# nanoporetech/taiyaki

Measured on AMD Instinct MI355X. Metric: signal-chunks/sec (T=4000) flip-flop train step, higher is better.
Workload: dtype f32; 1 GPU; configs[1]: mLstm_flipflop r9.4.1 DNA, chunk_len=4000 (T=800 blocks), 128 chunks/GPU, size 256, HIP flip-flop CRF loss + logZ, gradient maxima/clipping, AdamW; config_id=2, model=mLstm_flipflop, global_batch=128, chunk_len=4000, launch=hipGraph replay of forward+loss and of AdamW, eager backward, hw_queues=4, conv=gemm, lstm=miopen, batches=pre-assembled, cycled from HBM, parallelism=dp1 (reads sharded; one flat RCCL gradient all-reduce after backward)

## Files before the change

taiyaki_amd/csrc/lstm_fwd_layout.h:

```cpp
#pragma once

namespace tk {

constexpr bool lstm_fwd_lanes(int H, int U, int C) { return H == 256 && U == 64 && C == 2; }

struct LstmFwdLanes {
    int NT, H, U, C;
    int KP, KS, PR, CK;

    constexpr LstmFwdLanes(int nt, int h, int u, int c)
        : NT(nt), H(h), U(u), C(c), KP(nt / u), KS(h * u / nt), PR(c < 4 ? 4 / c : 1), CK(4 * c * u / nt) {}

    constexpr bool ok() const {
        return KP * U == NT && KS * KP == H && KP >= 4 && KP <= 64 && (KP & (KP - 1)) == 0 && PR >= 1 &&
               (PR * C) % 4 == 0 && KS % PR == 0 && CK >= 1 && CK * KP == 4 * C && C % CK == 0;
    }
    constexpr int k(int kp, int i) const { return i * KP + kp; }
    constexpr int hs_index(int k_, int c) const {
        return ((k_ / KP / PR) * KP + k_ % KP) * PR * C + (k_ / KP % PR) * C + c;
    }
    constexpr int chunk(int kp, int j) const { return (j * KP + kp) * PR * C; }
    constexpr int flat(int gate, int c) const { return (c / CK) * 4 * CK + gate * CK + c % CK; }
    constexpr int kept_first(int kp) const {
        int a = 0, n = 4 * C;
        for (int m = 1; m < KP; m <<= 1) {
            n /= 2;
            if (kp & m) a += n;
        }
        return a;
    }
    constexpr int gate(int kp) const { return kept_first(kp) % (4 * CK) / CK; }
    constexpr int col(int kp, int v) const { return kept_first(kp) / (4 * CK) * CK + v; }
    constexpr bool cell_lane(int kp) const { return gate(kp) == 0; }
    constexpr int gate_lane_xor(int g) const {
        for (int x = 0; x < KP; ++x)
            if (gate(x) == g && col(x, 0) == 0) return x;
        return -1;
    }
};

}
```

taiyaki_amd/csrc/lstm_kernels.hip:

```cpp
#include "dispatch.h"
#include "ff_common.h"
#include "lstm_bwd_layout.h"
#include "lstm_fwd_layout.h"
#include "rnn_common.h"

namespace tk {
namespace {

template <int U>
constexpr int threads_for() { return U == 48 ? 384 : U <= 32 ? 256 : 512; }
template <int H, int U>
constexpr int bwd_threads_for() { return U == 48 ? 2 * H : threads_for<U>(); }

template <int M>
__device__ __forceinline__ float xor_lane(float v) {
    static_assert(M == 1 || M == 2 || M == 4, "a partner inside the lane's group of 8");
    const int x = __float_as_int(v);
    if constexpr (M == 1) {
        return __int_as_float(__builtin_amdgcn_update_dpp(0, x, 0xB1, 0xF, 0xF, true));
    } else if constexpr (M == 2) {
        return __int_as_float(__builtin_amdgcn_update_dpp(0, x, 0x4E, 0xF, 0xF, true));
    } else {
        const int y = __builtin_amdgcn_update_dpp(0, x, 0x141, 0xF, 0xF, true);
        return __int_as_float(__builtin_amdgcn_update_dpp(0, y, 0x1B, 0xF, 0xF, true));
    }
}

template <int M, int RQ, int NA>
__device__ __forceinline__ void halve_rounds(float (&acc)[NA], int rq) {
    if constexpr (M < RQ) {
        constexpr int n = NA / (2 * M);
        const bool up = (rq & M) != 0;
#pragma unroll
        for (int a = 0; a < n; ++a) {
            const float send = up ? acc[a] : acc[a + n];
            const float keep = up ? acc[a + n] : acc[a];
            acc[a] = keep + xor_lane<M>(send);
        }
        halve_rounds<2 * M, RQ>(acc, rq);
    }
}

template <int H, int C, int U, bool VL, bool SAVE>
__device__ __forceinline__ void lstm_fwd_lanes_body(const float *__restrict__ gx, const float *__restrict__ whh, int T,
                                                    Cols cols, int reverse, int ngroups, float *__restrict__ y,
                                                    float *__restrict__ gates, float *__restrict__ cell, u64 *hbuf,
                                                    uint32_t *status, const int32_t *__restrict__ lengths) {
    constexpr int NT = threads_for<U>();
    const int N = cols.n, LD = cols.ld();
    constexpr int G = H / U;
    constexpr LstmFwdLanes FL(NT, H, U, C);
    constexpr int KP = FL.KP, KS = FL.KS, PR = FL.PR, CK = FL.CK;
    constexpr int NG = H * C / NT;
    static_assert(FL.ok() && KP == 8 && NG * NT == H * C && FL.gate_lane_xor(1) == 4 && FL.gate_lane_xor(2) == 2 &&
                      FL.gate_lane_xor(3) == 6,
                  "whole rows in 16-byte reads; the partial sums and the four gates of a column inside 8 lanes of a wave");
    constexpr int U4 = U / 4;
    constexpr int NQ = SAVE ? (6 * C * U4 + NT - 1) / NT : 1;
    static_assert(U % 4 == 0, "a row of the staging block is whole 16-byte chunks");
    __shared__ __attribute__((aligned(16))) float hs[2][H * C];
    __shared__ __attribute__((aligned(16))) float stg[SAVE ? 2 : 1][SAVE ? 6 * C * U : 4];
    __shared__ int give_up;

    int group, member;
    place(G, group, member);
    const int tid = threadIdx.x;
    const int j0 = member * U, n0 = group * C;
    const int u = tid / KP, kp = tid % KP;

    float w[4][KS];
#pragma unroll
    for (int g = 0; g < 4; ++g)
#pragma unroll
        for (int i = 0; i < KS; ++i) w[g][i] = whh[((size_t)g * H + j0 + u) * H + FL.k(kp, i)];
    settle(w);

    const int gate = FL.gate(kp), col = FL.col(kp, 0);
    const bool cell_lane = gate == 0;
    const int n = n0 + col;
    bool fetch[CK], valid[CK];
    float cst[CK], held[CK];
    int len[CK];
#pragma unroll
    for (int v = 0; v < CK; ++v) {
        fetch[v] = n + v < N;
        valid[v] = cell_lane && fetch[v];
        cst[v] = held[v] = 0.f;
        len[v] = 0;
        if constexpr (VL) len[v] = !valid[v] ? 0 : lengths ? lengths[n + v] : T;
    }

    for (int i = tid; i < H * C; i += NT) hs[0][i] = 0.f;
    if (tid == 0) give_up = 0;

    const size_t H4 = 4 * (size_t)H;
    float *rp[NQ];
    size_t rpitch[NQ];
    if constexpr (SAVE) {
#pragma unroll
        for (int i = 0; i < NQ; ++i) {
            const int q = tid + i * NT, row = q / U4, v = row / C, nn = n0 + row % C;
            const size_t w = v < 2 ? (size_t)H : H4;
            float *base = v == 0 ? y : v == 1 ? cell : gates + (size_t)(v - 2) * H;
            rpitch[i] = (size_t)LD * w;
            rp[i] = q < 6 * C * U4 && nn < N ? base + (size_t)nn * w + j0 + 4 * (q % U4) : nullptr;
        }
    }
    const float *gx0 = gx + (size_t)n * H4 + (size_t)gate * H + j0 + u;
    float gq[CK];
#pragma unroll
    for (int v = 0; v < CK; ++v) gq[v] = fetch[v] ? gx0[(size_t)(reverse ? T - 1 : 0) * LD * H4 + v * H4] : 0.f;
    __syncthreads();

    for (int s = 0; s < T; ++s) {
        const int t = reverse ? T - 1 - s : s;
        float *hb = hs[s & 1];
        settle(gq);
        if (s > 0) {
            const u64 *src = hbuf + ((size_t)((s - 1) & 1) * ngroups + group) * (H * C);
            float v[NG];
            if (!sweep<NG>(src, tid, NT, H * C, (unsigned)s, v, status)) give_up = 1;
#pragma unroll
            for (int q = 0; q < NG; ++q) {
                const int e = tid + q * NT;
                hb[FL.hs_index(e % H, e / H)] = v[q];
            }
            __syncthreads();
            if (give_up) return;
            const int tl = reverse ? t + 1 : t - 1;
            if constexpr (!SAVE) {
#pragma unroll
                for (int v = 0; v < CK; ++v)
                    if (valid[v]) y[((size_t)tl * LD + n + v) * H + j0 + u] = held[v];
            } else {
                rows_to_global<NQ>(stg[(s - 1) & 1], tid, NT, rp, rpitch, (size_t)tl);
            }
        }
        float gn[CK];
#pragma unroll
        for (int v = 0; v < CK; ++v)
            gn[v] = fetch[v] && s + 1 < T ? gx0[(size_t)(reverse ? t - 1 : t + 1) * LD * H4 + v * H4] : 0.f;
        asm volatile("" ::: "memory");

        float acc[4 * C];
#pragma unroll
        for (int a = 0; a < 4 * C; ++a) acc[a] = 0.f;
        constexpr int NR = KS / PR, AHEAD = 4;
        float hv[NR][PR * C];
#pragma unroll
        for (int j = 0; j < AHEAD; ++j) lds_row<PR * C>(hb + FL.chunk(kp, j), hv[j]);
#pragma unroll
        for (int j = 0; j < NR; ++j) {
            if (j + AHEAD < NR) lds_row<PR * C>(hb + FL.chunk(kp, j + AHEAD), hv[j + AHEAD]);
            __builtin_amdgcn_sched_barrier(0);
#pragma unroll
            for (int e = 0; e < PR; ++e)
#pragma unroll
                for (int g = 0; g < 4; ++g)
#pragma unroll
                    for (int c = 0; c < C; ++c)
                        acc[FL.flat(g, c)] = fmaf(w[g][PR * j + e], hv[j][e * C + c], acc[FL.flat(g, c)]);
        }
        halve_rounds<1, KP>(acc, kp);

        float ig[CK], fg[CK], gg[CK], og[CK];
#pragma unroll
        for (int v = 0; v < CK; ++v) {
            const float x = acc[v] + gq[v];
            float a;
            if (gate == 2)
                a = tanhf(x);
            else
                a = sigmoidf(x);
            ig[v] = a;
            gg[v] = xor_lane<2>(a);
            fg[v] = xor_lane<4>(a);
            og[v] = xor_lane<2>(fg[v]);
        }

        if (cell_lane) {
            float h[CK];
#pragma unroll
            for (int v = 0; v < CK; ++v) {
                cst[v] = fmaf(ig[v], gg[v], fg[v] * cst[v]);
                h[v] = og[v] * tanhf(cst[v]);
                if constexpr (VL) {
                    if (t >= len[v]) {
                        cst[v] = h[v] = 0.f;
                        if constexpr (SAVE) ig[v] = fg[v] = gg[v] = og[v] = 0.f;
                    }
                }
            }
            if (s + 1 < T) {
#pragma unroll
                for (int v = 0; v < CK; ++v)
                    store_granule(hbuf + ((size_t)(s & 1) * ngroups + group) * (H * C) + (col + v) * H + j0 + u,
                                  (unsigned)(s + 1), h[v]);
            }
#pragma unroll
            for (int v = 0; v < CK; ++v) {
                if constexpr (!SAVE) {
                    held[v] = h[v];
                } else {
                    float *sp = stg[s & 1] + (col + v) * U + u;
                    sp[0 * C * U] = h[v];
                    sp[1 * C * U] = cst[v];
                    sp[2 * C * U] = ig[v];
                    sp[3 * C * U] = fg[v];
                    sp[4 * C * U] = gg[v];
                    sp[5 * C * U] = og[v];
                }
            }
        }
#pragma unroll
        for (int v = 0; v < CK; ++v) gq[v] = gn[v];
    }
    if (T > 0) {
        const int tl = reverse ? 0 : T - 1;
        if constexpr (!SAVE) {
#pragma unroll
            for (int v = 0; v < CK; ++v)
                if (valid[v]) y[((size_t)tl * LD + n + v) * H + j0 + u] = held[v];
        } else {
            __syncthreads();
            rows_to_global<NQ>(stg[(T - 1) & 1], tid, NT, rp, rpitch, (size_t)tl);
        }
    }
}

template <int H, int C, int U, bool VL = false, bool SAVE = !VL>
__global__ __launch_bounds__(threads_for<U>(), 1) void lstm_fwd_kernel(const float *__restrict__ gx,
                                                                       const float *__restrict__ whh, int T, Cols cols,
                                                                       int reverse, int ngroups,
                                                                       float *__restrict__ y,
                                                                       float *__restrict__ gates,
                                                                       float *__restrict__ cell, u64 *hbuf,
                                                                       uint32_t *status,
                                                                       const int32_t *__restrict__ lengths) {
    if constexpr (lstm_fwd_lanes(H, U, C)) {
        lstm_fwd_lanes_body<H, C, U, VL, SAVE>(gx, whh, T, cols, reverse, ngroups, y, gates, cell, hbuf, status, lengths);
        return;
    }
    constexpr int NT = threads_for<U>();
    const int N = cols.n, LD = cols.ld();
    constexpr int G = H / U;
    constexpr int KP = NT / U;
    constexpr int KS = H / KP;
    constexpr int NG = (H * C + NT - 1) / NT;
    static_assert(KS >= 1 && KP <= 64 && C <= KP, "lane (u, kp) inside one wave; one cell lane per (u, column)");
    constexpr int U4 = U / 4;
    constexpr int NQ = SAVE ? (6 * C * U4 + NT - 1) / NT : 1;
    static_assert(U % 4 == 0, "a row of the staging block is whole 16-byte chunks");
    __shared__ __attribute__((aligned(16))) float hs[2][H * C];
    __shared__ __attribute__((aligned(16))) float stg[SAVE ? 2 : 1][SAVE ? 6 * C * U : 4];
    __shared__ int give_up;

    int group, member;
    place(G, group, member);
    const int tid = threadIdx.x;
    const int j0 = member * U, n0 = group * C;
    const int u = tid / KP, kp = tid % KP;

    float w[4][KS];
#pragma unroll
    for (int g = 0; g < 4; ++g)
#pragma unroll
        for (int i = 0; i < KS; ++i) w[g][i] = whh[((size_t)g * H + j0 + u) * H + i * KP + kp];
    settle(w);

    int col = 0;
#pragma unroll
    for (int m = 1, width = C; width > 1; m <<= 1, width >>= 1)
        if (kp & m) col += width / 2;
    const bool cell_lane = kp < C;
    const int n = n0 + col;
    const bool valid = cell_lane && n < N;
    float cst = 0.f;
    int len = 0;
    if constexpr (VL) len = !valid ? 0 : lengths ? lengths[n] : T;

    for (int i = tid; i < H * C; i += NT) hs[0][i] = 0.f;
    if (tid == 0) give_up = 0;

    const size_t H4 = 4 * (size_t)H;
    float *rp[NQ];
    size_t rpitch[NQ];
    if constexpr (SAVE) {
#pragma unroll
        for (int i = 0; i < NQ; ++i) {
            const int q = tid + i * NT, row = q / U4, v = row / C, nn = n0 + row % C;
            const size_t w = v < 2 ? (size_t)H : H4;
            float *base = v == 0 ? y : v == 1 ? cell : gates + (size_t)(v - 2) * H;
            rpitch[i] = (size_t)LD * w;
            rp[i] = q < 6 * C * U4 && nn < N ? base + (size_t)nn * w + j0 + 4 * (q % U4) : nullptr;
        }
    }
    float gq[4] = {0.f, 0.f, 0.f, 0.f};
    if (valid) {
        const float *p = gx + ((size_t)(reverse ? T - 1 : 0) * LD + n) * H4 + j0 + u;
#pragma unroll
        for (int g = 0; g < 4; ++g) gq[g] = p[(size_t)g * H];
    }
    float held = 0.f;
    __syncthreads();

    for (int s = 0; s < T; ++s) {
        const int t = reverse ? T - 1 - s : s;
        float *hb = hs[s & 1];
        settle(gq);
        if (s > 0) {
            const u64 *src = hbuf + ((size_t)((s - 1) & 1) * ngroups + group) * (H * C);
            float v[NG];
            if (!sweep<NG>(src, tid, NT, H * C, (unsigned)s, v, status)) give_up = 1;
#pragma unroll
            for (int q = 0; q < NG; ++q) {
                const int e = tid + q * NT;
                if (e < H * C) hb[(e % H) * C + e / H] = v[q];
            }
            __syncthreads();
            if (give_up) return;
            const int tl = reverse ? t + 1 : t - 1;
            if constexpr (!SAVE) {
                if (valid) y[((size_t)tl * LD + n) * H + j0 + u] = held;
            } else {
                rows_to_global<NQ>(stg[(s - 1) & 1], tid, NT, rp, rpitch, (size_t)tl);
            }
        }
        float gn[4] = {0.f, 0.f, 0.f, 0.f};
        if (valid && s + 1 < T) {
            const float *p = gx + ((size_t)(reverse ? t - 1 : t + 1) * LD + n) * H4 + j0 + u;
#pragma unroll
            for (int g = 0; g < 4; ++g) gn[g] = p[(size_t)g * H];
        }
        asm volatile("" ::: "memory");

        float acc[4][C];
#pragma unroll
        for (int g = 0; g < 4; ++g)
#pragma unroll
            for (int c = 0; c < C; ++c) acc[g][c] = 0.f;
#pragma unroll
        for (int i = 0; i < KS; ++i) {
            float hv[C];
            lds_row<C>(hb + (i * KP + kp) * C, hv);
#pragma unroll
            for (int g = 0; g < 4; ++g)
#pragma unroll
                for (int c = 0; c < C; ++c) acc[g][c] = fmaf(w[g][i], hv[c], acc[g][c]);
        }
#pragma unroll
        for (int m = 1; m < KP; m <<= 1) {
            const int half = C / (2 * m);
            const bool up = (kp & m) != 0;
#pragma unroll
            for (int g = 0; g < 4; ++g) {
                if (half == 0) acc[g][0] += __shfl_xor(acc[g][0], m);
#pragma unroll
                for (int c = 0; c < C / 2; ++c) {
                    if (c < half) {
                        const float send = up ? acc[g][c] : acc[g][c + half];
                        const float keep = up ? acc[g][c + half] : acc[g][c];
                        acc[g][c] = keep + __shfl_xor(send, m);
                    }
                }
            }
        }

        if (cell_lane) {
            float ig = sigmoidf(acc[0][0] + gq[0]), fg = sigmoidf(acc[1][0] + gq[1]);
            float gg = tanhf(acc[2][0] + gq[2]), og = sigmoidf(acc[3][0] + gq[3]);
            cst = fmaf(ig, gg, fg * cst);
            float h = og * tanhf(cst);
            if constexpr (VL) {
                if (t >= len) {
                    cst = h = 0.f;
                    if constexpr (SAVE) ig = fg = gg = og = 0.f;
                }
            }
            if (s + 1 < T)
                store_granule(hbuf + ((size_t)(s & 1) * ngroups + group) * (H * C) + col * H + j0 + u,
                              (unsigned)(s + 1), h);
            if constexpr (!SAVE) {
                held = h;
            } else {
                float *sp = stg[s & 1] + col * U + u;
                sp[0 * C * U] = h;
                sp[1 * C * U] = cst;
                sp[2 * C * U] = ig;
                sp[3 * C * U] = fg;
                sp[4 * C * U] = gg;
                sp[5 * C * U] = og;
            }
        }
#pragma unroll
        for (int g = 0; g < 4; ++g) gq[g] = gn[g];
    }
    if (T > 0) {
        const int tl = reverse ? 0 : T - 1;
        if constexpr (!SAVE) {
            if (valid) y[((size_t)tl * LD + n) * H + j0 + u] = held;
        } else {
            __syncthreads();
            rows_to_global<NQ>(stg[(T - 1) & 1], tid, NT, rp, rpitch, (size_t)tl);
        }
    }
}

#ifndef TK_RNN_VARLEN
template <int H, int C, int U, bool VL = false>
__global__ __launch_bounds__((bwd_threads_for<H, U>()), 1) void lstm_bwd_kernel(const float *__restrict__ whh,
                                                                       const float *__restrict__ gates,
                                                                       const float *__restrict__ cell,
                                                                       const float *__restrict__ dy, int T, Cols cols,
                                                                       int reverse, int ngroups,
                                                                       float *__restrict__ dgates, u64 *pbuf,
                                                                       uint32_t *status,
                                                                       const int32_t *__restrict__ lengths) {
    constexpr int NT = bwd_threads_for<H, U>();
    const int N = cols.n, LD = cols.ld();
    constexpr int G = H / U;
    constexpr bool STRIDED = U == 48;
    constexpr int RP = NT / H;
    constexpr int R = 4 * U / RP;
    constexpr LstmBwdBlock LB(NT, H, U, C);
    constexpr bool BLOCK = LB.KQ > 0;
    constexpr int KQ = BLOCK ? LB.KQ : 1, RQ = BLOCK ? LB.RQ : 1, RR = BLOCK ? LB.RR : 1, KEEP = BLOCK ? LB.KEEP : 1;
    constexpr int PAIRS = U * C;
    constexpr int PL = NT / PAIRS;
    constexpr int NP = (G + PL - 1) / PL;
    constexpr bool APART = BLOCK && NP > 1;
    static_assert(!APART || NP * PL == G, "every plane polls NP producers");
    static_assert(RP >= 1 && R >= 1 && PL >= 1 && PL * PAIRS == NT, "every lane polls; one cell lane per pair");
    static_assert(!STRIDED || (RP * H == NT && R * RP == 4 * U && U % RP == 0),
                  "a lane's rows keep their gate index at compile time");
    static_assert(!BLOCK || (LB.ok() && KQ * RR * NT == 4 * U * H && RQ <= 64 && (RQ & (RQ - 1)) == 0 &&
                             KEEP * NT == C * H && KQ * RR == R),
                  "every owned weight in one lane; the RQ partial sums inside one wave; one granule per held sum");
    __shared__ __attribute__((aligned(16))) float dgs[4 * U * C];
    __shared__ float gath[(APART ? G : PL) * PAIRS];
    __shared__ __attribute__((aligned(16))) float red[RP > 1 && !BLOCK ? RP * C * H : 1];
    __shared__ int give_up;

    int group, member;
    place(G, group, member);
    const int tid = threadIdx.x;
    const int j0 = member * U, n0 = group * C;

    const int k = tid % H, rp = tid / H;
    const int kb = tid / RQ, rq = tid % RQ;
    float w[R];
    if constexpr (BLOCK) {
#pragma unroll
        for (int j = 0; j < RR; ++j) {
            const int r = LB.row(rq, j);
#pragma unroll
            for (int q = 0; q < KQ; ++q) w[q * RR + j] = whh[((size_t)(r / U) * H + j0 + (r % U)) * H + KQ * kb + q];
        }
    } else if constexpr (STRIDED) {
        const float *wbase = whh + (size_t)(j0 + rp) * H + k;
#pragma unroll
        for (int i = 0; i < R; ++i) w[i] = wbase[(unsigned)((((i * RP) / U) * H + (i * RP) % U) * H)];
    } else {
#pragma unroll
        for (int i = 0; i < R; ++i) {
            const int r = rp * R + i;
            w[i] = whh[((size_t)(r / U) * H + j0 + (r % U)) * H + k];
        }
    }
    settle(w);

    const bool cell_lane = tid < PAIRS;
    const int pair = tid % PAIRS, plane = tid / PAIRS;
    const int cc = pair / U, u = pair % U;
    const int n = n0 + cc;
    const bool valid = cell_lane && n < N;
    float dc_next = 0.f, f_next = 0.f;
    int len = 0;
    if constexpr (VL) len = !valid ? 0 : lengths ? lengths[n] : T;
    if (tid == 0) give_up = 0;

    const size_t H4 = 4 * (size_t)H;
    float in[7] = {0.f, 0.f, 0.f, 0.f, 0.f, 0.f, 0.f};
    if (valid) {
        const int t = reverse ? 0 : T - 1;
        const size_t o = ((size_t)t * LD + n) * H + j0 + u;
        in[0] = dy[o];
        in[1] = cell[o];
        if (T > 1) in[2] = cell[((size_t)(reverse ? t + 1 : t - 1) * LD + n) * H + j0 + u];
        const float *gp = gates + ((size_t)t * LD + n) * H4 + j0 + u;
#pragma unroll
        for (int g = 0; g < 4; ++g) in[3 + g] = gp[(size_t)g * H];
    }
    float held[4] = {0.f, 0.f, 0.f, 0.f};
    __syncthreads();

    const u64 *mine = pbuf + (size_t)group * G * C * H + cc * H + j0 + u;
    const int a0 = LB.kept_first(rq), pub = (a0 % C) * H + KQ * kb + a0 / C;
    for (int s = 0; s < T; ++s) {
        const int tt = T - 1 - s;
        const int t = reverse ? T - 1 - tt : tt;
        const int tp = reverse ? t + 1 : t - 1;
        settle(in);
        float dhr = 0.f;
        if (s > 0) {
            float v[NP];
            const int nvalid = plane < G ? (G - plane + PL - 1) / PL : 0;
            const u64 *src = mine + (size_t)((s - 1) & 1) * ngroups * G * C * H;
            if (!sweep<NP>(src, plane * C * H, PL * C * H, G * C * H, (unsigned)s, v, status)) give_up = 1;
            if constexpr (APART) {
#pragma unroll
                for (int q = 0; q < NP; ++q) gath[(plane + q * PL) * PAIRS + pair] = v[q];
            } else {
                float sum = 0.f;
#pragma unroll
                for (int q = 0; q < NP; ++q)
                    if (q < nvalid) sum += v[q];
                gath[plane * PAIRS + pair] = sum;
            }
            __syncthreads();
            if (give_up) return;
            if (cell_lane) {
#pragma unroll
                for (int p = 0; p < (APART ? G : PL); ++p) dhr += gath[p * PAIRS + pair];
            }
            if (valid) {
                const int tl = reverse ? t - 1 : t + 1;
                float *dp = dgates + ((size_t)tl * LD + n) * H4 + j0 + u;
#pragma unroll
                for (int g = 0; g < 4; ++g) dp[(size_t)g * H] = held[g];
            }
        }
        float nx[7] = {0.f, 0.f, 0.f, 0.f, 0.f, 0.f, 0.f};
        if (valid && tt > 0) {
            const size_t o = ((size_t)tp * LD + n) * H + j0 + u;
            nx[0] = dy[o];
            nx[1] = in[2];
            if (tt > 1) nx[2] = cell[((size_t)(reverse ? tp + 1 : tp - 1) * LD + n) * H + j0 + u];
            const float *gp = gates + ((size_t)tp * LD + n) * H4 + j0 + u;
#pragma unroll
            for (int g = 0; g < 4; ++g) nx[3 + g] = gp[(size_t)g * H];
        }
        asm volatile("" ::: "memory");

        if (cell_lane) {
            const float ct = in[1];
            float cp = in[2];
            if constexpr (VL) {
                if (tp >= len) cp = 0.f;
            }
            const float ig = in[3], gg = in[5], og = in[6];
            float fg = in[4];
            const float dh = in[0] + dhr;
            const float tc = tanhf(ct);
            float dc = dh * og * (1.f - tc * tc) + dc_next * f_next;
            float di = dc * gg * ig * (1.f - ig);
            float df = dc * cp * fg * (1.f - fg);
            float dg = dc * ig * (1.f - gg * gg);
            float dout = dh * tc * og * (1.f - og);
            if constexpr (VL) {
                if (t >= len) dc = fg = di = df = dg = dout = 0.f;
            }
            dc_next = dc;
            f_next = fg;
            held[0] = di;
            held[1] = df;
            held[2] = dg;
            held[3] = dout;
            dgs[(0 * U + u) * C + cc] = valid ? di : 0.f;
            dgs[(1 * U + u) * C + cc] = valid ? df : 0.f;
            dgs[(2 * U + u) * C + cc] = valid ? dg : 0.f;
            dgs[(3 * U + u) * C + cc] = valid ? dout : 0.f;
        }
#pragma unroll
        for (int q = 0; q < 7; ++q) in[q] = nx[q];
        __syncthreads();
        if (s + 1 == T) break;

        if constexpr (BLOCK) {
            u64 *dst = pbuf + (((size_t)(s & 1) * ngroups + group) * G + member) * C * H;
            float acc[KQ * C];
#pragma unroll
            for (int a = 0; a < KQ * C; ++a) acc[a] = 0.f;
#pragma unroll
            for (int i = 0; i < RR / 2; ++i) {
                float d[2 * C];
                lds_row<2 * C>(dgs + (rq + RQ * i) * 2 * C, d);
#pragma unroll
                for (int e = 0; e < 2; ++e)
#pragma unroll
                    for (int q = 0; q < KQ; ++q)
#pragma unroll
                        for (int c = 0; c < C; ++c)
                            acc[q * C + c] = fmaf(w[q * RR + 2 * i + e], d[e * C + c], acc[q * C + c]);
            }
            halve_rounds<1, RQ>(acc, rq);
#pragma unroll
            for (int v = 0; v < KEEP; ++v) store_granule(dst + pub + v * H, (unsigned)(s + 1), acc[v]);
            continue;
        }
        float acc[C];
#pragma unroll
        for (int c = 0; c < C; ++c) acc[c] = 0.f;
#pragma unroll
        for (int i = 0; i < R; ++i) {
            float d[C];
            lds_row<C>(dgs + (STRIDED ? i * RP + rp : rp * R + i) * C, d);
#pragma unroll
            for (int c = 0; c < C; ++c) acc[c] = fmaf(w[i], d[c], acc[c]);
        }
        u64 *dst = pbuf + (((size_t)(s & 1) * ngroups + group) * G + member) * C * H;
        if constexpr (RP == 1) {
#pragma unroll
            for (int c = 0; c < C; ++c) store_granule(dst + c * H + k, (unsigned)(s + 1), acc[c]);
        } else {
#pragma unroll
            for (int c = 0; c < C; ++c) red[(rp * C + c) * H + k] = acc[c];
            __syncthreads();
            for (int e = tid; e < C * H; e += NT) {
                float v = 0.f;
#pragma unroll
                for (int q = 0; q < RP; ++q) v += red[q * C * H + e];
                store_granule(dst + e, (unsigned)(s + 1), v);
            }
        }
    }
    if (valid && T > 0) {
        const int tl = reverse ? T - 1 : 0;
        float *dp = dgates + ((size_t)tl * LD + n) * H4 + j0 + u;
#pragma unroll
        for (int g = 0; g < 4; ++g) dp[(size_t)g * H] = held[g];
    }
}

#endif

int g_lab_cols = 0;
int g_lab_units = 0;

int units48(size_t H) { return H == 192 || H == 384 ? 48 : 0; }

bool lstm_geometry(size_t N, size_t H, int cu_count, int *C_out, int *groups_out) {
    const int U48 = units48(H);
    if (!(U48 || H == 16 || H == 32 || H == 64 || H == 128 || H == 256) || N == 0 || cu_count <= 0) return false;
    const size_t G = H / (U48 ? U48 : 16);
    const int first = U48 ? 4 : 8, last = H == 384 ? 4 : 2 * first;
    for (int C = first; C <= last; C *= 2) {
        if (g_lab_cols != 0 && C != g_lab_cols) continue;
        const size_t groups = (N + C - 1) / C;
        if (groups * G <= (size_t)cu_count) {
            *C_out = C;
            *groups_out = (int)groups;
            return true;
        }
    }
    return false;
}

size_t ws_bytes(size_t H, int C, int groups, int U, bool backward) {
    return 2 * (size_t)groups * (backward ? H / U : 1) * C * H * sizeof(u64);
}

struct Plan {
    int U, C, groups;
    unsigned grid;
};

bool lstm_plan(size_t N, size_t H, int cu_count, Plan *p) {
    int C16 = 0, groups16 = 0;
    if (!lstm_geometry(N, H, cu_count, &C16, &groups16)) return false;
    if (const int U48 = units48(H)) {
        *p = Plan{U48, C16, groups16, (unsigned)(groups16 * (H / U48))};
        return true;
    }
    int U = g_lab_units != 0 ? g_lab_units : 64;
    if ((size_t)U > H) U = (int)H;
    if (U != 16 && U != 32 && U != 64) return false;
    p->U = U;
    p->C = C16 * 16 / U;
    p->groups = (int)((N + p->C - 1) / p->C);
    p->grid = (unsigned)(p->groups * (H / U));
    return true;
}

#define TK_LSTM_SWITCH(LAUNCH)                                                                                    \
    switch ((int)H * 100000 + p.U * 1000 + p.C) {                                                                 \
        LAUNCH(16, 16, 8) LAUNCH(16, 16, 16) LAUNCH(32, 16, 8) LAUNCH(32, 16, 16) LAUNCH(64, 16, 8)                \
        LAUNCH(64, 16, 16) LAUNCH(128, 16, 8) LAUNCH(128, 16, 16) LAUNCH(256, 16, 8) LAUNCH(256, 16, 16)          \
        LAUNCH(32, 32, 4) LAUNCH(32, 32, 8) LAUNCH(64, 32, 4) LAUNCH(64, 32, 8) LAUNCH(128, 32, 4)                 \
        LAUNCH(128, 32, 8) LAUNCH(256, 32, 4) LAUNCH(256, 32, 8)                                                  \
        LAUNCH(64, 64, 2) LAUNCH(64, 64, 4) LAUNCH(128, 64, 2) LAUNCH(128, 64, 4) LAUNCH(256, 64, 2)               \
        LAUNCH(256, 64, 4) LAUNCH(192, 48, 4) LAUNCH(192, 48, 8) LAUNCH(384, 48, 4)                               \
        default: return TK_ERR_UNSUPPORTED;                                                                       \
    }

template <bool VL, bool SAVE>
int launch_fwd(const Plan &p, size_t H, hipStream_t st, const float *gx, const float *whh, int T, Cols cols,
               int rev, float *y, float *gates, float *cell, u64 *ws, uint32_t *status, const int32_t *lengths) {
#define TK_LSTM_FWD(HH, UU, CC)                                                                                  \
    case HH * 100000 + UU * 1000 + CC:                                                                           \
        hipLaunchKernelGGL((lstm_fwd_kernel<HH, CC, UU, VL, SAVE>), dim3(p.grid), dim3(threads_for<UU>()), 0, st, gx,  \
                           whh, T, cols, rev, p.groups, y, gates, cell, ws, status, lengths);                    \
        break;
    TK_LSTM_SWITCH(TK_LSTM_FWD)
#undef TK_LSTM_FWD
    return hipGetLastError() == hipSuccess ? TK_OK : TK_ERR_LAUNCH;
}

#ifndef TK_RNN_VARLEN
template <bool VL>
int launch_bwd(const Plan &p, size_t H, hipStream_t st, const float *whh, const float *gates, const float *cell,
               const float *dy, int T, Cols cols, int rev, float *dg, u64 *ws, uint32_t *status,
               const int32_t *lengths) {
#define TK_LSTM_BWD(HH, UU, CC)                                                                                   \
    case HH * 100000 + UU * 1000 + CC:                                                                            \
        hipLaunchKernelGGL((lstm_bwd_kernel<HH, CC, UU, VL>), dim3(p.grid), dim3(bwd_threads_for<HH, UU>()), 0,   \
                           st, whh, gates, cell, dy, T, cols, rev, p.groups, dg, ws, status, lengths);            \
        break;
    TK_LSTM_SWITCH(TK_LSTM_BWD)
#undef TK_LSTM_BWD
    return hipGetLastError() == hipSuccess ? TK_OK : TK_ERR_LAUNCH;
}
#endif
#undef TK_LSTM_SWITCH

size_t lstm_slab(size_t N, size_t H, int cu_count) {
    int C = 0, groups = 0;
    const size_t S = widest_admitted([&](size_t n) { return lstm_geometry(n, H, cu_count, &C, &groups); });
    return N == 0 ? 0 : N < S ? N : S;
}

template <class Launch>
int checked(bool pointers_ok, size_t T, size_t N, size_t H, int cu_count, void *ws, size_t wsb, uint32_t *status,
            hipStream_t stream, bool backward, Launch launch) {
    if (!pointers_ok || !ws || !status || !aligned16(ws) || T > (size_t)INT32_MAX || N > (size_t)INT32_MAX)
        return TK_ERR_BAD_ARG;
#ifdef TK_RNN_WIDE
    const size_t S = lstm_slab(N, H, cu_count);
#else
    const size_t S = N;
#endif
    if (S == 0) return TK_ERR_UNSUPPORTED;
    for (size_t first = 0; first < N; first += S) {
        const size_t n = N - first < S ? N - first : S;
        Plan p;
        if (!lstm_plan(n, H, cu_count, &p)) return TK_ERR_UNSUPPORTED;
        const size_t need = ws_bytes(H, p.C, p.groups, p.U, backward);
        if (wsb < need) return TK_ERR_WORKSPACE;
        if (T == 0) continue;
        int rc = zero_ws(ws, need, stream);
        if (rc != TK_OK) return rc;
        rc = launch(p, first, make_cols(n, N));
        if (rc != TK_OK) return rc;
    }
    return TK_OK;
}

size_t train_workspace_bytes(size_t N, size_t H, int cu_count) {
    int C = 0, groups = 0;
    if (!lstm_geometry(N, H, cu_count, &C, &groups)) return 0;
    const int U48 = units48(H);
    return ws_bytes(H, C, groups, U48 ? U48 : 16, true);
}

template <bool VL, bool SAVE>
int forward(const float *gx, const float *whh, const int32_t *lengths, size_t T, size_t N, size_t H, int reverse,
            int cu_count, float *y, float *gates, float *cell, void *ws, size_t wsb, uint32_t *status,
            hipStream_t stream) {
    auto launch = [&](const Plan &p, size_t first, Cols cols) {
        return launch_fwd<VL, SAVE>(p, H, stream, at_column(gx, first, 4 * H), whh, (int)T, cols, reverse,
                                    at_column(y, first, H), at_column(gates, first, 4 * H), at_column(cell, first, H),
                                    static_cast<u64 *>(ws), status, at_column(lengths, first, 1));
    };
    return checked(gx && whh && y && (!SAVE || (gates && cell)), T, N, H, cu_count, ws, wsb, status, stream, false,
                   launch);
}

#ifndef TK_RNN_VARLEN
template <bool VL>
int backward(const float *whh, const float *gates, const float *cell, const float *dy, const int32_t *lengths,
             size_t T, size_t N, size_t H, int reverse, int cu_count, float *dgates, void *ws, size_t wsb,
             uint32_t *status, hipStream_t stream) {
    auto launch = [&](const Plan &p, size_t first, Cols cols) {
        return launch_bwd<VL>(p, H, stream, whh, at_column(gates, first, 4 * H), at_column(cell, first, H),
                              at_column(dy, first, H), (int)T, cols, reverse, at_column(dgates, first, 4 * H),
                              static_cast<u64 *>(ws), status, at_column(lengths, first, 1));
    };
    return checked(whh && gates && cell && dy && dgates, T, N, H, cu_count, ws, wsb, status, stream, true, launch);
}
#endif

}

#ifdef TK_RNN_VARLEN
size_t lstm_varlen_workspace_bytes(size_t N, size_t H, int cu_count) {
    Plan p;
    if (!lstm_plan(N, H, cu_count, &p)) return 0;
    return ws_bytes(H, p.C, p.groups, p.U, false);
}

int lstm_forward_varlen_dispatch(const float *gx, const float *whh, const int32_t *lengths, size_t T, size_t N,
                                 size_t H, int reverse, int cu_count, float *y, void *ws, size_t wsb,
                                 uint32_t *status, hipStream_t stream) {
    return forward<true, false>(gx, whh, lengths, T, N, H, reverse, cu_count, y, nullptr, nullptr, ws, wsb, status,
                                stream);
}
#elif defined(TK_RNN_VARLEN_TRAIN)
size_t lstm_varlen_train_workspace_bytes(size_t N, size_t H, int cu_count) {
    return train_workspace_bytes(N, H, cu_count);
}

int lstm_forward_varlen_save_dispatch(const float *gx, const float *whh, const int32_t *lengths, size_t T, size_t N,
                                      size_t H, int reverse, int cu_count, float *y, float *gates, float *cell,
                                      void *ws, size_t wsb, uint32_t *status, hipStream_t stream) {
    return forward<true, true>(gx, whh, lengths, T, N, H, reverse, cu_count, y, gates, cell, ws, wsb, status, stream);
}

int lstm_backward_varlen_dispatch(const float *whh, const float *gates, const float *cell, const float *dy,
                                  const int32_t *lengths, size_t T, size_t N, size_t H, int reverse, int cu_count,
                                  float *dgates, void *ws, size_t wsb, uint32_t *status, hipStream_t stream) {
    return backward<true>(whh, gates, cell, dy, lengths, T, N, H, reverse, cu_count, dgates, ws, wsb, status, stream);
}
#elif defined(TK_RNN_WIDE)
size_t lstm_wide_slab(size_t N, size_t H, int cu_count) { return lstm_slab(N, H, cu_count); }

size_t lstm_wide_workspace_bytes(size_t N, size_t H, int cu_count) {
    return train_workspace_bytes(lstm_slab(N, H, cu_count), H, cu_count);
}

int lstm_forward_wide_dispatch(const float *gx, const float *whh, const int32_t *lengths, size_t T, size_t N,
                               size_t H, int reverse, int cu_count, float *y, float *gates, float *cell, void *ws,
                               size_t wsb, uint32_t *status, hipStream_t stream) {
    if (!gates != !cell) return TK_ERR_BAD_ARG;
    return gates ? forward<true, true>(gx, whh, lengths, T, N, H, reverse, cu_count, y, gates, cell, ws, wsb, status,
                                       stream)
                 : forward<true, false>(gx, whh, lengths, T, N, H, reverse, cu_count, y, nullptr, nullptr, ws, wsb,
                                        status, stream);
}

int lstm_backward_wide_dispatch(const float *whh, const float *gates, const float *cell, const float *dy,
                                const int32_t *lengths, size_t T, size_t N, size_t H, int reverse, int cu_count,
                                float *dgates, void *ws, size_t wsb, uint32_t *status, hipStream_t stream) {
    return backward<true>(whh, gates, cell, dy, lengths, T, N, H, reverse, cu_count, dgates, ws, wsb, status, stream);
}
#else
size_t lstm_workspace_bytes(size_t N, size_t H, int cu_count) { return train_workspace_bytes(N, H, cu_count); }

int lstm_forward_dispatch(const float *gx, const float *whh, size_t T, size_t N, size_t H, int reverse,
                          int cu_count, float *y, float *gates, float *cell, void *ws, size_t wsb,
                          uint32_t *status, hipStream_t stream) {
    return forward<false, true>(gx, whh, nullptr, T, N, H, reverse, cu_count, y, gates, cell, ws, wsb, status, stream);
}

int lstm_backward_dispatch(const float *whh, const float *gates, const float *cell, const float *dy, size_t T,
                           size_t N, size_t H, int reverse, int cu_count, float *dgates, void *ws, size_t wsb,
                           uint32_t *status, hipStream_t stream) {
    return backward<false>(whh, gates, cell, dy, nullptr, T, N, H, reverse, cu_count, dgates, ws, wsb, status, stream);
}

#ifdef TK_LAB
void lstm_lab_cols(int cols) { g_lab_cols = cols; }
void lstm_lab_units(int units) { g_lab_units = units; }

bool lstm_lab_geometry(size_t N, size_t H, int cu_count, size_t *out) {
    int C16 = 0, groups16 = 0;
    Plan p;
    if (!lstm_geometry(N, H, cu_count, &C16, &groups16) || !lstm_plan(N, H, cu_count, &p)) return false;
    const size_t v[8] = {(size_t)C16, (size_t)groups16, (size_t)p.U, (size_t)p.C, (size_t)p.groups, p.grid,
                         ws_bytes(H, p.C, p.groups, p.U, false), ws_bytes(H, p.C, p.groups, p.U, true)};
    for (int i = 0; i < 8; ++i) out[i] = v[i];
    return true;
}
#endif
#endif

}
```

Measured before the change: 5230 chunks/s.

## Split LSTM forward workgroup into two interleaved column sets with staggered polling

Adds a specialized forward LSTM body for H=256, U=64, C=2 with saved activations. Each half of the workgroup owns one batch column and the two columns alternate within each time step. While one half computes its recurrent matvec, the other polls the cross-workgroup hidden-state exchange and writes its saved rows, so global latency hides behind compute. The cost is a more intricate schedule with more barriers per step and a new lane layout that has to stay consistent with the exchange protocol.

```diff
diff --git a/taiyaki_amd/csrc/lstm_fwd_layout.h b/taiyaki_amd/csrc/lstm_fwd_layout.h
--- a/taiyaki_amd/csrc/lstm_fwd_layout.h
+++ b/taiyaki_amd/csrc/lstm_fwd_layout.h
@@ -39,4 +39,36 @@
     }
 };
 
+constexpr bool lstm_fwd_two_sets(int H, int U, int C, bool VL, bool SAVE) {
+    return lstm_fwd_lanes(H, U, C) && !VL && SAVE;
 }
+
+struct LstmFwdSet {
+    int NT, H, U;
+    int KP, KS, PR;
+
+    constexpr LstmFwdSet(int nt, int h, int u) : NT(nt), H(h), U(u), KP(nt / u), KS(h * u / nt), PR(4) {}
+
+    constexpr bool ok() const { return KP * U == NT && KS * KP == H && KP == 8 && KS % PR == 0 && 2 * H == NT; }
+    constexpr int k(int kp, int i) const { return i * KP + kp; }
+    constexpr int hs_index(int k_) const { return ((k_ / KP / PR) * KP + k_ % KP) * PR + k_ / KP % PR; }
+    constexpr int chunk(int kp, int j) const { return (j * KP + kp) * PR; }
+    constexpr int kept(int kp) const {
+        int a = 0, n = 4;
+        for (int m = 1; m < 4; m <<= 1) {
+            n /= 2;
+            if (kp & m) a += n;
+        }
+        return a;
+    }
+    constexpr int gate(int kp) const { return kept(kp); }
+    constexpr bool cell_lane(int kp) const { return kp == 0; }
+    constexpr int gate_lane_xor(int g) const {
+        for (int x = 0; x < KP; ++x)
+            if (gate(x) == g) return x;
+        return -1;
+    }
+    constexpr int poll_role(int tid) const { return tid / H; }
+};
+
+}
diff --git a/taiyaki_amd/csrc/lstm_kernels.hip b/taiyaki_amd/csrc/lstm_kernels.hip
--- a/taiyaki_amd/csrc/lstm_kernels.hip
+++ b/taiyaki_amd/csrc/lstm_kernels.hip
@@ -228,6 +228,165 @@
     }
 }
 
+template <int H, int C, int U>
+__device__ __forceinline__ void lstm_fwd_two_sets_body(const float *__restrict__ gx, const float *__restrict__ whh, int T,
+                                                       Cols cols, int reverse, int ngroups, float *__restrict__ y,
+                                                       float *__restrict__ gates, float *__restrict__ cell, u64 *hbuf,
+                                                       uint32_t *status) {
+    constexpr int NT = threads_for<U>();
+    const int N = cols.n, LD = cols.ld();
+    constexpr int G = H / U;
+    constexpr LstmFwdSet FS(NT, H, U);
+    constexpr int KP = FS.KP, KS = FS.KS, PR = FS.PR;
+    constexpr int U4 = U / 4, NCH = 6 * U4;
+    static_assert(C == 2 && FS.ok() && FS.gate_lane_xor(1) == 2 && FS.gate_lane_xor(2) == 1 && FS.gate_lane_xor(3) == 3 &&
+                      NCH <= H && U % 4 == 0,
+                  "two sets of one column; a set's granules one per lane of half the workgroup; f, g, o inside the quad");
+    __shared__ __attribute__((aligned(16))) float hs[2][2][H];
+    __shared__ __attribute__((aligned(16))) float stg[2][2][6 * U];
+    __shared__ int give_up;
+
+    int group, member;
+    place(G, group, member);
+    const int tid = threadIdx.x;
+    const int j0 = member * U, n0 = group * C;
+    const int u = tid / KP, kp = tid % KP;
+    const int role = __builtin_amdgcn_readfirstlane(FS.poll_role(tid));
+    const int li = tid % H;
+
+    float w[4][KS];
+#pragma unroll
+    for (int g = 0; g < 4; ++g)
+#pragma unroll
+        for (int i = 0; i < KS; ++i) w[g][i] = whh[((size_t)g * H + j0 + u) * H + FS.k(kp, i)];
+    settle(w);
+
+    const int gate = FS.gate(kp);
+    const bool cell_lane = FS.cell_lane(kp);
+    const bool fetch[2] = {n0 < N, n0 + 1 < N};
+    float cst[2] = {0.f, 0.f};
+
+    for (int i = tid; i < 2 * 2 * H; i += NT) (&hs[0][0][0])[i] = 0.f;
+    if (tid == 0) give_up = 0;
+
+    const size_t H4 = 4 * (size_t)H;
+    float *rp = nullptr;
+    size_t rpitch = 0;
+    if (li < NCH && n0 + (1 - role) < N) {
+        const int v = li / U4;
+        const size_t wd = v < 2 ? (size_t)H : H4;
+        float *base = v == 0 ? y : v == 1 ? cell : gates + (size_t)(v - 2) * H;
+        rpitch = (size_t)LD * wd;
+        rp = base + (size_t)(n0 + (1 - role)) * wd + j0 + 4 * (li % U4);
+    }
+    const float *gx0 = gx + (size_t)n0 * H4 + (size_t)gate * H + j0 + u;
+    auto gx_at = [&](int X, int sn) {
+        const int tn = reverse ? T - 1 - sn : sn;
+        return fetch[X] && sn < T ? gx0[(size_t)tn * LD * H4 + X * H4] : 0.f;
+    };
+    float gq[2] = {gx_at(0, 0), 0.f};
+    float gn[2][2] = {{gx_at(0, 0), gx_at(1, 0)}, {gx_at(0, 1), gx_at(1, 0)}};
+    settle(gq);
+    settle(gn);
+    u64 early[2] = {0, 0};
+    __syncthreads();
+
+    for (int s = 0; s < T; ++s) {
+#pragma unroll
+        for (int X = 0; X < 2; ++X) {
+            float *hb = hs[X][s & 1];
+            if (role == X) {
+                if (s > 0) {
+                    const u64 e = early[X];
+                    float v[1] = {__uint_as_float((unsigned)e)};
+                    if (!__all((unsigned)(e >> 32) == (unsigned)s)) {
+                        const u64 *src = hbuf + ((size_t)((s - 1) & 1) * ngroups + group) * (H * C) + X * H;
+                        if (!sweep<1>(src, li, H, H, (unsigned)s, v, status)) give_up = 1;
+                    }
+                    hb[FS.hs_index(li)] = v[0];
+                }
+                settle(gn[X]);
+                gq[0] = gn[X][0];
+                gq[1] = gn[X][1];
+            }
+            __syncthreads();
+            if (give_up) return;
+            if (role == X) {
+                settle(gn[X]);
+                const int sb = X == 0 ? s - 1 : s;
+                if (sb >= 0 && rp) {
+                    const float4 q = reinterpret_cast<const float4 *>(stg[1 - X][sb & 1])[li];
+                    *reinterpret_cast<row_chunk *>(rp + (size_t)(reverse ? T - 1 - sb : sb) * rpitch) =
+                        row_chunk{q.x, q.y, q.z, q.w};
+                }
+                gn[X][X] = gx_at(X, s + 1);
+                gn[X][1 - X] = gx_at(1 - X, s + 1 + X);
+            }
+            asm volatile("" ::: "memory");
+
+            float acc[4] = {0.f, 0.f, 0.f, 0.f};
+            constexpr int NR = KS / PR, AHEAD = 4;
+            float hv[NR][PR];
+#pragma unroll
+            for (int j = 0; j < AHEAD; ++j) lds_row<PR>(hb + FS.chunk(kp, j), hv[j]);
+#pragma unroll
+            for (int j = 0; j < NR; ++j) {
+                if (j + AHEAD < NR) lds_row<PR>(hb + FS.chunk(kp, j + AHEAD), hv[j + AHEAD]);
+                __builtin_amdgcn_sched_barrier(0);
+#pragma unroll
+                for (int e = 0; e < PR; ++e)
+#pragma unroll
+                    for (int g = 0; g < 4; ++g) acc[g] = fmaf(w[g][PR * j + e], hv[j][e], acc[g]);
+            }
+            halve_rounds<1, 4>(acc, kp);
+            acc[0] = acc[0] + xor_lane<4>(acc[0]);
+
+            if (role == 1 - X) {
+                const int sp = s + X;
+                if (sp > 0 && sp < T)
+                    early[1 - X] = __hip_atomic_load(
+                        (gu64 *)(hbuf + ((size_t)((sp - 1) & 1) * ngroups + group) * (H * C) + (1 - X) * H + li),
+                        __ATOMIC_RELAXED, __HIP_MEMORY_SCOPE_AGENT);
+            }
+            __builtin_amdgcn_sched_barrier(0);
+
+            const float x = acc[0] + gq[X];
+            float ig;
+            if (gate == 2)
+                ig = tanhf(x);
+            else
+                ig = sigmoidf(x);
+            const float gg = xor_lane<1>(ig);
+            const float fg = xor_lane<2>(ig);
+            const float og = xor_lane<1>(fg);
+            float h = 0.f;
+            if ((kp & 3) == 0) {
+                cst[X] = fmaf(ig, gg, fg * cst[X]);
+                h = og * tanhf(cst[X]);
+            }
+            h = __int_as_float(__builtin_amdgcn_update_dpp(0, __float_as_int(h), 0x00, 0xF, 0xF, true));
+            store_granule(hbuf + ((size_t)(s & 1) * ngroups + group) * (H * C) + X * H + j0 + u, (unsigned)(s + 1), h);
+            asm volatile("" ::: "memory");
+            if (cell_lane) {
+                float *sp = stg[X][s & 1] + u;
+                sp[0 * U] = h;
+                sp[1 * U] = cst[X];
+                sp[2 * U] = ig;
+                sp[3 * U] = fg;
+                sp[4 * U] = gg;
+                sp[5 * U] = og;
+            }
+        }
+    }
+    if (T > 0) {
+        __syncthreads();
+        if (role == 0 && rp) {
+            const float4 q = reinterpret_cast<const float4 *>(stg[1][(T - 1) & 1])[li];
+            *reinterpret_cast<row_chunk *>(rp + (size_t)(reverse ? 0 : T - 1) * rpitch) = row_chunk{q.x, q.y, q.z, q.w};
+        }
+    }
+}
+
 template <int H, int C, int U, bool VL = false, bool SAVE = !VL>
 __global__ __launch_bounds__(threads_for<U>(), 1) void lstm_fwd_kernel(const float *__restrict__ gx,
                                                                        const float *__restrict__ whh, int T, Cols cols,
@@ -237,6 +396,10 @@
                                                                        float *__restrict__ cell, u64 *hbuf,
                                                                        uint32_t *status,
                                                                        const int32_t *__restrict__ lengths) {
+    if constexpr (lstm_fwd_two_sets(H, U, C, VL, SAVE)) {
+        lstm_fwd_two_sets_body<H, C, U>(gx, whh, T, cols, reverse, ngroups, y, gates, cell, hbuf, status);
+        return;
+    }
     if constexpr (lstm_fwd_lanes(H, U, C)) {
         lstm_fwd_lanes_body<H, C, U, VL, SAVE>(gx, whh, T, cols, reverse, ngroups, y, gates, cell, hbuf, status, lengths);
         return;
```

Result: no change. 5260 chunks/s (median of 6 runs) (+0.6%).
